# fjdf/slaMEM

Measured on AMD Instinct MI355X. Metric: MEMs/sec (and queries/sec) on 100 Mbp ref x 10 M 150 bp queries, l=20, higher is better.
Workload: dtype u32; 1 GPU; synthetic 100000000 bp reference (splitmix64 seed 42) x 10000000 reads/GPU of 150 bp, 2% substitutions, 50% reverse-complemented, -b -l 20; ref_len=100000000, reads_total=10000000, read_len=150, min_len=20, both_strands=True, parallelism=query shards x1, one GPU, no replication

## Files before the change

### slamem_amd/csrc/mem_search.hip

```cpp
#include "common.h"
#include "prims.h"

#include <atomic>
#include <type_traits>
#include <new>
#include <stdlib.h>
#include <string.h>

namespace slamem {

struct Blk {
    uint4 a;
    uint4 b;
    uint4 c;
    uint4 d;
};

__device__ __forceinline__ uint64_t u64_of(uint32_t lo, uint32_t hi) { return ((uint64_t)hi << 32) | lo; }

__device__ __forceinline__ Blk load_blk(const FMBlock* __restrict__ fm, uint32_t bi) {
    const uint4* p = reinterpret_cast<const uint4*>(fm + bi);
    Blk k;
    k.a = p[0]; k.b = p[1]; k.c = p[2]; k.d = p[3];
    return k;
// ... 1773 lines not shown
    const uint32_t a = sl * kSliceLen;
    if (!(slen >= k && slen - a >= 1u)) return 0;
    const uint32_t b = slen - a < kSliceLen ? slen : a + kSliceLen;
    auto win = [&](uint32_t p, uint32_t len, bool& has_n) -> uint64_t {
        const uint64_t v = span_letters(pk, nm, rel + (rev ? slen - p - len : p), len, has_n);
        if (rev) return ~v & ((1ull << (2u * len)) - 1ull);
        uint64_t r = __brevll(v) >> (64u - 2u * len);
        return ((r & 0x5555555555555555ull) << 1) | ((r >> 1) & 0x5555555555555555ull);
    };
    auto present = [&](const uint64_t* line, uint64_t h) -> bool {
        const uint64_t bits = kfilter_bits(h);
        return (line[kfilter_word(h)] & bits) == bits;
    };
    uint8_t res = 0;
    bool hn;
    if (s <= 6u) {
        const uint32_t k1 = k - 2u, s1 = L - k1 + 1u;
        const bool three = L >= k + 2u && k + 2u <= 32u && ix.kfilter_levels >= 3u;
        const uint32_t p0 = (a + s1 - 1u) / s1 * s1;
        const uint32_t pmax = (uint32_t)(((uint64_t)b + s1 - 2u < (uint64_t)(slen - k1)) ? b + s1 - 2u : slen - k1);
#pragma unroll 1
        for (uint32_t p = p0; p <= pmax && !res; p += s1) {
            const uint64_t v1 = win(p, k1, hn);
            if (hn) { res = 1; break; }
            const uint64_t h1 = kfilter_hash(v1 ^ kFilterShortSalt);
            const uint64_t* line = ix.kfilter + kfilter_line(h1, ix.kfilter_log2);
            if (kStats) n_probe++;
            if (!present(line, h1)) continue;
#pragma unroll 1
            for (uint32_t t = 0; t < 3u && !res; t++) {
                if (p + t < 2u || (uint64_t)p + t - 2u + k > slen) continue;
                const uint32_t q = p + t - 2u;
                const uint64_t vk = win(q, k, hn);
                if (hn) { res = 1; break; }
                if (!present(line, kfilter_hash(vk))) continue;
                if (!three) { res = 1; break; }
#pragma unroll 1
                for (uint32_t u = 0; u < 3u && !res; u++) {
                    if (q + u < 2u || (uint64_t)q + u + k > slen) continue;
                    const uint64_t v3 = win(q + u - 2u, k + 2u, hn);
                    if (hn) { res = 1; break; }
                    if (present(line, kfilter_hash(v3 ^ kFilterLongSalt))) res = 1;
                }
            }
        }
    } else {
        const uint32_t p0 = (a + s - 1u) / s * s;
        const uint32_t pmax = (uint32_t)(((uint64_t)b + s - 2u < (uint64_t)(slen - k)) ? b + s - 2u : slen - k);
#pragma unroll 1
        for (uint32_t p = p0; p <= pmax && !res; p += s) {
            const uint64_t vk = win(p, k, hn);
            if (hn) { res = 1; break; }
            const uint64_t* line = ix.kfilter + kfilter_line(kfilter_hash((vk >> 4) ^ kFilterShortSalt), ix.kfilter_log2);
            if (kStats) n_probe++;
            if (!present(line, kfilter_hash(vk))) continue;
            if (k + 2u > 32u || ix.kfilter_levels < 3u) { res = 1; break; }
#pragma unroll 1
            for (uint32_t u = 0; u < 3u && !res; u++) {
                if (p + u < 2u || (uint64_t)p + u + k > slen) continue;
                const uint64_t v3 = win(p + u - 2u, k + 2u, hn);
                if (hn || present(line, kfilter_hash(v3 ^ kFilterLongSalt))) res = 1;
            }
        }
    }
    return res;
}

template <bool kStats>
__device__ __forceinline__ uint8_t prefilter_item(const SearchArgs& A, const ItemDesc& d, uint32_t& n_probe, uint32_t& n_qload) {
    const IndexView& ix = A.ix;
    const uint32_t k = ix.kfilter_k, L = A.min_len;
    const uint32_t s = L - k + 1u;
    uint32_t sl = d.slice_rev & 0x7FFFFFFFu;
    uint32_t a = sl * kSliceLen;
    uint32_t b = d.len - a < kSliceLen ? d.len : a + kSliceLen;
    uint8_t res = 0;
    if (d.len >= k && d.len - a >= 1u && s <= 6u) {
        const uint32_t k1 = k - 2u, s1 = L - k1 + 1u;
        const uint32_t p0 = (a + s1 - 1u) / s1 * s1;
        uint32_t pmax = (uint32_t)(((uint64_t)b + s1 - 2u < (uint64_t)(d.len - k1)) ? b + s1 - 2u : d.len - k1);
        if (p0 <= pmax) {
            QueryStream qs;
            const bool three = L >= k + 2u && k + 2u <= 32u && ix.kfilter_levels >= 3u;
            const uint32_t kw = three ? k + 2u : k;
            const uint64_t mask = kw >= 32u ? ~0ull : (1ull << (2u * kw)) - 1ull;
            const uint64_t maskk = (1ull << (2u * k)) - 1ull, mask1 = (1ull << (2u * k1)) - 1ull;
            uint64_t km = 0;
            uint32_t run = 0, confirm = 0, confirm2 = 0;
            const uint64_t* line1 = ix.kfilter;
            const uint64_t* line2 = ix.kfilter;
            uint32_t x = p0 >= 4u ? p0 - 4u : 0u;
            qs.init(A.qwords, d.base, d.len, d.slice_rev >> 31, x);
            uint64_t xe64 = (uint64_t)pmax + k1 + 1u + (three ? 2u : 0u);
            const uint32_t xend = xe64 > (uint64_t)d.len - 1u ? d.len - 1u : (uint32_t)xe64;
            uint32_t wend = p0 + k1 - 1u;
            const uint32_t wlast = pmax + k1 - 1u;
            for (; x <= xend && !res; x++) {
                uint32_t c = qs.next();
                if (c >= 2u) { km = ((km << 2) | (uint64_t)(c - 2u)) & mask; run++; }
                else { km = 0; run = 0; }
                if (x == wend && wend <= wlast) {
                    wend += s1;
                    if (run < k1) res = 1;
                    else {
                        uint64_t h = kfilter_hash((km & mask1) ^ kFilterShortSalt), bits = kfilter_bits(h);
                        if (kStats) n_probe++;
                        line1 = ix.kfilter + kfilter_line(h, ix.kfilter_log2);
                        if ((line1[kfilter_word(h)] & bits) == bits) confirm = 3;
                    }
                }
                if (confirm && !res) {
                    confirm--;
                    if (x + 1u >= k) {
                        if (run < k) res = 1;
                        else {
                            uint64_t h = kfilter_hash(km & maskk), bits = kfilter_bits(h);
                            if ((line1[kfilter_word(h)] & bits) == bits) {
                                if (three) { confirm2 = 3; line2 = line1; }
                                else res = 1;
                            }
                        }
                    }
                }
                if (confirm2 && !res) {
                    confirm2--;
                    if (x + 1u >= k + 2u) {
                        if (run < k + 2u) res = 1;
                        else {
                            uint64_t h = kfilter_hash(km ^ kFilterLongSalt), bits = kfilter_bits(h);
                            if ((line2[kfilter_word(h)] & bits) == bits) res = 1;
                        }
                    }
                }
            }
            if (kStats) n_qload += qs.loads;
        }
    } else if (d.len >= k && d.len - a >= 1u) {
        const uint32_t p0 = (a + s - 1u) / s * s;
        const uint32_t pmax = (uint32_t)(((uint64_t)b + s - 2u < (uint64_t)(d.len - k)) ? b + s - 2u : d.len - k);
        if (p0 <= pmax) {
            QueryStream qs;
            qs.init(A.qwords, d.base, d.len, d.slice_rev >> 31, p0);
            const uint64_t mask = (1ull << (2u * k)) - 1ull;
            uint64_t km = 0;
            uint32_t run = 0, wend = p0 + k - 1u;
            const uint32_t xend = pmax + k - 1u;
            for (uint32_t x = p0; x <= xend && !res; x++) {
                uint32_t c = qs.next();
                if (c >= 2u) { km = ((km << 2) | (uint64_t)(c - 2u)) & mask; run++; }
                else { km = 0; run = 0; }
                if (x == wend) {
                    wend += s;
                    if (run < k) res = 1;
                    else {
                        const uint64_t* line = ix.kfilter + kfilter_line(kfilter_hash((km >> 4) ^ kFilterShortSalt), ix.kfilter_log2);
                        uint64_t h = kfilter_hash(km), bits = kfilter_bits(h);
                        if (kStats) n_probe++;
                        if ((line[kfilter_word(h)] & bits) == bits) res = 1;
                    }
                }
            }
            if (kStats) n_qload += qs.loads;
        }
    }
    return res;
}

#ifndef SLAMEM_PF_WAVES
#define SLAMEM_PF_WAVES 8
#endif
template <bool kStats>
__global__ void __launch_bounds__(256, SLAMEM_PF_WAVES) k_prefilter(SearchArgs A, uint8_t* __restrict__ alive) {
    uint64_t g = (uint64_t)blockIdx.x * blockDim.x + threadIdx.x;
    const bool live = g < A.num_items;
    if (!live) g = 0;
    uint32_t n_probe = 0, n_qload = 0;
    ItemDesc d = A.items[g];
    if (!live) d.len = 0;
    uint8_t res;
    if (kPfStageChunks != 0u) {
        __shared__ uint32_t s_pk[kPfStageChunks + 2u];
        __shared__ uint16_t s_nm[kPfStageChunks + 2u];
        __shared__ unsigned long long s_lo[4], s_hi[4];
        unsigned long long lo = d.len ? d.base >> 4 : ~0ull, hi = d.len ? ((d.base + d.len - 1u) >> 4) + 1ull : 0ull;
#pragma unroll
        for (int o = 32; o; o >>= 1) {
            unsigned long long l2 = __shfl_xor(lo, o), h2 = __shfl_xor(hi, o);
            lo = l2 < lo ? l2 : lo;
            hi = h2 > hi ? h2 : hi;
        }
        if ((threadIdx.x & 63u) == 0u) { s_lo[threadIdx.x >> 6] = lo; s_hi[threadIdx.x >> 6] = hi; }
        __syncthreads();
#pragma unroll
        for (int w = 0; w < 4; w++) {
            lo = s_lo[w] < lo ? s_lo[w] : lo;
            hi = s_hi[w] > hi ? s_hi[w] : hi;
        }
        auto pack_span = [&](unsigned long long first_chunk, uint32_t n) {
            const uint4* src = reinterpret_cast<const uint4*>(A.qwords) + first_chunk;
#pragma unroll 1
            for (uint32_t i = threadIdx.x; i < n; i += 256u) {
                uint32_t pk, nm;
                pack_chunk(src[i], pk, nm);
                s_pk[i] = pk;
                s_nm[i] = (uint16_t)nm;
                if (kStats) n_qload++;
            }
            if (threadIdx.x < 2u) { s_pk[n + threadIdx.x] = 0u; s_nm[n + threadIdx.x] = 0u; }
            __syncthreads();
        };
        if (hi > lo && hi - lo <= (unsigned long long)kPfStageChunks) {
            pack_span(lo, (uint32_t)(hi - lo));
            res = prefilter_item_packed<kStats>(A, d, s_pk, s_nm, (uint32_t)(d.base - (lo << 4)), n_probe);
        } else {
            auto span_lo = [&](uint32_t first, uint32_t count) {
                unsigned long long v = ~0ull;
                for (uint32_t w = first; w < first + count; w++) v = s_lo[w] < v ? s_lo[w] : v;
                return v;
            };
            auto span_hi = [&](uint32_t first, uint32_t count) {
                unsigned long long v = 0ull;
                for (uint32_t w = first; w < first + count; w++) v = s_hi[w] > v ? s_hi[w] : v;
                return v;
            };
            uint32_t per_part = 0u;
            for (uint32_t cnt = 2u; cnt >= 1u && !per_part; cnt >>= 1) {
                bool fits = true;
                for (uint32_t first = 0; first < 4u; first += cnt) {
                    const unsigned long long l = span_lo(first, cnt), h = span_hi(first, cnt);
                    if (h > l && h - l > (unsigned long long)kPfStageChunks) fits = false;
                }
                if (fits) per_part = cnt;
            }
            if (per_part && hi > lo) {
                const uint32_t my_wave = threadIdx.x >> 6;
                res = 0;
#pragma unroll 1
                for (uint32_t first = 0; first < 4u; first += per_part) {
                    lo = span_lo(first, per_part);
                    hi = span_hi(first, per_part);
                    if (hi <= lo) continue;
                    __syncthreads();
                    pack_span(lo, (uint32_t)(hi - lo));
                    if (my_wave >= first && my_wave < first + per_part)
                        res = prefilter_item_packed<kStats>(A, d, s_pk, s_nm, (uint32_t)(d.base - (lo << 4)), n_probe);
                }
            } else {
                res = prefilter_item<kStats>(A, d, n_probe, n_qload);
            }
        }
    } else {
        res = prefilter_item<kStats>(A, d, n_probe, n_qload);
    }
    if (live) alive[g] = res;
    if (kStats) {
        stat_flush<kStats>(A.stats + SC_PF_PROBES, n_probe);
        stat_flush<kStats>(A.stats + SC_PF_QUERY_LOADS, n_qload);
        stat_flush<kStats>(A.stats + SC_PF_ITEMS, live ? 1u : 0u);
    }
}

__global__ void __launch_bounds__(256) k_prefilter_list(SearchArgs A, const uint32_t* __restrict__ list, const uint32_t* __restrict__ list_count,
                                                        uint8_t* __restrict__ alive) {
    const uint32_t count = *list_count;
    for (uint32_t i = blockIdx.x * blockDim.x + threadIdx.x; i < count; i += gridDim.x * blockDim.x) {
        const uint32_t g = list[i];
        const ItemDesc d = item_of(A, g);
        uint32_t n_probe = 0, n_qload = 0;
        if (!prefilter_item<false>(A, d, n_probe, n_qload)) alive[g] = 0;
    }
}

#ifndef SLAMEM_SEED_READS
#define SLAMEM_SEED_READS 21
#endif
constexpr uint32_t kSeedReads = SLAMEM_SEED_READS, kSeedReadsMid = 16, kSeedReadsLong = 16;
constexpr uint32_t kSeedMaxLen = 192;
constexpr uint32_t kSeedMaxLenMid = 256;
constexpr uint32_t kSeedMaxLenLong = 384;
#ifndef SLAMEM_SEED_JOBS
#define SLAMEM_SEED_JOBS 16
#endif
constexpr uint32_t kSeedJobs = SLAMEM_SEED_JOBS;
#ifndef SLAMEM_SEED_MEMS
#define SLAMEM_SEED_MEMS 12
#endif
constexpr uint32_t kSeedMems = SLAMEM_SEED_MEMS;
constexpr uint32_t kSigLetters = 12, kSigMask = (1u << kSigLetters) - 1u, kSigKnown = 1u << 24;

template <uint32_t NW, uint32_t R>
struct SeedWave {
    static constexpr uint32_t kJobs = kSeedJobs * R * NW / 3u, kMems = kSeedMems * R * NW / 3u;
    uint64_t pl[R][2][2][NW + 1];
    uint32_t len[R];
    uint32_t nwin[R];
    union {
        uint4 raw[R * NW * 4 + 1];
        struct {
            uint32_t job_p[kJobs], job_x[kJobs];
            uint32_t mem_key[kMems], mem_ref[kMems];
            uint32_t mem_sig[kMems];
        };
    };
    uint32_t bad[R];
    uint64_t pn[R][NW + 1];
    uint32_t hasn;
    unsigned long long expl[R];
    union {
        uint16_t ring[128];
        unsigned long long smask[2 * R];
    };
    uint32_t flags;
    uint32_t pad[3];
};

__device__ __forceinline__ void wave_sync() {
    __builtin_amdgcn_fence(__ATOMIC_RELEASE, "wavefront");
    __builtin_amdgcn_wave_barrier();
    __builtin_amdgcn_fence(__ATOMIC_ACQUIRE, "wavefront");
}
__device__ __forceinline__ uint64_t funnel64(uint64_t lo, uint64_t hi, uint32_t sh) { return (lo >> sh) | ((hi << 1) << (63u - sh)); }
__device__ __forceinline__ uint64_t bits_below(int x) {
    const int c = x < 0 ? 0 : x > 64 ? 64 : x;
    return c == 0 ? 0ull : (~0ull >> (64 - c));
}
__device__ __forceinline__ uint64_t bits_range(int lo, int hi) { return bits_below(hi) & ~bits_below(lo); }
__device__ __forceinline__ uint32_t sel4(const uint4& v, uint32_t a) {
    const uint32_t lo = (a & 1u) ? v.y : v.x, hi = (a & 1u) ? v.w : v.z;
    return (a & 2u) ? hi : lo;
}
__device__ __forceinline__ uint32_t sel12(const uint4& b0, const uint4& b1, const uint4& b2, uint32_t e) {
    const uint32_t a = e & 3u, x0 = sel4(b0, a), x1 = sel4(b1, a), x2 = sel4(b2, a);
    return e < 4u ? x0 : e < 8u ? x1 : x2;
}
__device__ __forceinline__ uint32_t byte_tops(uint32_t m) {
    const uint32_t y = m >> 7;
    return (y | (y >> 7) | (y >> 14) | (y >> 21)) & 0xFu;
}

#ifndef SLAMEM_SEED_WAVES
#define SLAMEM_SEED_WAVES 1
#endif
template <bool kStats, uint32_t NW, uint32_t R>
__global__ void __launch_bounds__(256, SLAMEM_SEED_WAVES) k_seed_mems(SearchArgs A, uint8_t* __restrict__ alive) {
    constexpr uint32_t kMaxLen = 64u * NW;
    static_assert(R <= 32u && R * NW <= 128u, "a flag word holds a bit per read; the planes step runs in at most two passes");
    __shared__ SeedWave<NW, R> lds[4];
    const IndexView& ix = A.ix;
    const uint32_t lane = threadIdx.x & 63u, wv = threadIdx.x >> 6;
    SeedWave<NW, R>& S = lds[wv];
    const uint32_t strands = A.strands, k = ix.seed_k, L = A.min_len, s = L - k + 1u;
    const uint32_t kmask = (1u << k) - 1u;
    const uint64_t r0 = ((uint64_t)blockIdx.x * 4u + wv) * R;
    if (r0 >= (uint64_t)A.num_queries) return;
    const uint32_t nr = (uint64_t)A.num_queries - r0 < R ? (uint32_t)((uint64_t)A.num_queries - r0) : R;
    const unsigned long long below = (1ull << lane) - 1ull;
    const int64_t ulast = (int64_t)text_units(ix.n) - 1;
    uint32_t n_win = 0, n_cmp = 0, n_nm = 0, n_mem = 0;

    const uint64_t off = lane <= nr ? A.offsets[r0 + lane] : 0ull;
    constexpr uint32_t kRawChunks = R * NW * 4u + 1u, kSpecIters = (kRawChunks + 63u) / 64u;
#ifndef SLAMEM_SEED_NO_SPEC
    constexpr bool kSpec = kSpecIters <= 5u;
#else
    constexpr bool kSpec = false;
#endif
    uint4 sv[kSpec ? kSpecIters : 1u];
    uint64_t g0 = 0, len0 = 0;
    bool spec = false;
    if (kSpec) {
        const uint64_t o0 = A.offsets[0], o1 = A.offsets[1], o_end = A.offsets[A.num_queries];
        len0 = o1 - o0;
        g0 = o0 + r0 * len0;
        const uint64_t g1 = g0 + (uint64_t)nr * len0;
        spec = len0 != 0ull && len0 <= (uint64_t)kMaxLen && g1 <= o_end;
        const uint32_t gn = spec ? (uint32_t)(((g1 - 1u) >> 4) - (g0 >> 4) + 1u) : 0u;
        const uint4* src = reinterpret_cast<const uint4*>(A.qwords) + (g0 >> 4);
#pragma unroll
        for (uint32_t j = 0; j < kSpecIters; j++) {
            const uint32_t c = lane + 64u * j;
            sv[j] = c < gn ? src[c] : make_uint4(0, 0, 0, 0);
        }
    }
    const uint64_t offn = __shfl_down(off, 1);
    if (kSpec) spec = spec && __ballot(lane <= nr && off != g0 + (uint64_t)lane * len0) == 0ull;
    uint32_t len = 0, nwin = 0;
    bool left = false;
    if (lane < nr) {
        const uint64_t l64 = offn - off;
        if (l64 > kSliceLen) atomicOr(A.seed_long_flag, 1u);
        if (l64 > kMaxLen) left = l64 >= L; else len = (uint32_t)l64;
        if (len >= L) nwin = (len - k) / s + 1u;
        if (nwin > 64u) { left = true; nwin = 0; }
    }
#ifndef SLAMEM_SEED_NO_FORM_HINT
    const uint32_t lg_grid = 31u - (uint32_t)__clz((int)(gridDim.x | 1u));
    if ((blockIdx.x & ((1u << (lg_grid > 8u ? lg_grid - 8u : 0u)) - 1u)) == 0u) {
        const uint64_t l64 = lane < nr ? offn - off : 0ull;
        if (lane == 0u) atomicAdd(A.seed_wide + 3, nr);
        if (NW < 6u) {
            const bool w4 = NW < 4u && l64 > kMaxLen && l64 <= kSeedMaxLenMid && l64 >= L;
            const bool w6 = l64 > (kMaxLen > kSeedMaxLenMid ? kMaxLen : kSeedMaxLenMid) && l64 <= kSeedMaxLenLong && l64 >= L;
            const uint32_t n4 = (uint32_t)__popcll(__ballot(w4)), n6 = (uint32_t)__popcll(__ballot(w6));
            if (lane == 0u && n4) atomicAdd(A.seed_wide, n4);
            if (lane == 0u && n6) atomicAdd(A.seed_wide + 1, n6);
        }
        if (NW > 3u) {
            const bool needed = l64 > (NW == 4u ? kSeedMaxLen : kSeedMaxLenMid) && l64 <= kMaxLen;
            if (__ballot(needed) != 0ull && lane == 0u) A.seed_wide[2] = 1u;
        }
    }
#endif
    uint32_t wflags = (uint32_t)__ballot(left);
    if (lane == 0u) S.flags = 0u;
    const uint32_t plen = nwin ? len : 0u;
    const uint64_t span0 = u64_of((uint32_t)__builtin_amdgcn_readlane((int)(uint32_t)off, 0), (uint32_t)__builtin_amdgcn_readlane((int)(uint32_t)(off >> 32), 0));
    const uint64_t span1 = u64_of((uint32_t)__builtin_amdgcn_readlane((int)(uint32_t)off, (int)nr), (uint32_t)__builtin_amdgcn_readlane((int)(uint32_t)(off >> 32), (int)nr));
    const uint64_t chunk0 = span0 >> 4;
    const uint32_t nchunks = span1 > span0 ? (uint32_t)(((span1 - 1u) >> 4) - chunk0 + 1u) : 0u;
    const bool staged = nchunks <= kRawChunks;
    if (kSpec && spec) {
#pragma unroll
        for (uint32_t j = 0; j < kSpecIters; j++) {
            const uint32_t c = lane + 64u * j;
            if (c < nchunks) S.raw[c] = sv[kSpec ? j : 0u];
        }
    } else if (staged) {
        const uint4* src = reinterpret_cast<const uint4*>(A.qwords) + chunk0;
        for (uint32_t c = lane; c < nchunks; c += 64u) S.raw[c] = src[c];
    }
    wave_sync();
    if (lane < R) S.bad[lane] = 0u;
    if (lane == 0u) S.hasn = 0u;
    const bool text_pure = ix.num_n == 0u;
    wave_sync();
    const uint32_t* rawwords = reinterpret_cast<const uint32_t*>(S.raw);
    const uint32_t* qw32 = reinterpret_cast<const uint32_t*>(A.qwords);
    const uint64_t qlast32 = ((A.offsets[A.num_queries] + 7ull) >> 3) * 2ull - 1ull;
    constexpr uint32_t kRawLast = (R * NW * 4u + 1u) * 4u - 1u;
    for (uint32_t pb = 0; pb < nr * NW; pb += 64u) {
        const uint32_t pp = pb + lane, i = pp / NW, j = pp % NW;
        const bool on = pp < nr * NW;
        const uint32_t Li = __shfl(plen, (int)(on ? i : 0u));
        const uint64_t base = __shfl(off, (int)(on ? i : 0u));
        if (on && 64u * j < Li) {
            const uint32_t nv = Li - 64u * j < 64u ? Li - 64u * j : 64u;
            const uint64_t a = base + 64u * j;
            const uint32_t sh8 = (uint32_t)(a & 3u);
            uint32_t w[17];
            if (staged) {
                const uint32_t i0 = (uint32_t)((a - (chunk0 << 4)) >> 2);
#pragma unroll
                for (uint32_t t = 0; t < 17u; t++) w[t] = rawwords[i0 + t < kRawLast ? i0 + t : kRawLast];
            } else {
                const uint64_t i0 = a >> 2;
#pragma unroll
                for (uint32_t t = 0; t < 17u; t++) w[t] = qw32[i0 + t < qlast32 ? i0 + t : qlast32];
            }
            uint32_t p0lo = 0, p0hi = 0, p1lo = 0, p1hi = 0, bad = 0;
#pragma unroll
            for (uint32_t t = 0; t < 16u; t++) {
                const uint32_t d = __builtin_amdgcn_alignbyte(w[t + 1u], w[t], sh8);
                const uint32_t nb = nv > 4u * t ? (nv - 4u * t < 4u ? nv - 4u * t : 4u) : 0u;
                const uint32_t M = nb >= 4u ? 0x01010101u : (0x01010101u & ((1u << (8u * nb)) - 1u));
                const uint32_t B0 = d, B1 = d >> 1, B2 = d >> 2, B3 = d >> 3, B4 = d >> 4, B6 = d >> 6, B7 = d >> 7;
                const uint32_t tt = B2 & ~B1, good = (B0 ^ tt) & ~((B4 ^ tt) | B3 | B7) & B6;
                bad |= ~good & M;
                const uint32_t X = ((B1 ^ B2) & M) | ((B2 & M) << 4);
                const uint32_t G = (X | (X >> 7) | (X >> 14) | (X >> 21)) & 0xFFu;
                if (t < 8u) { p0lo |= (G & 0xFu) << (4u * t); p1lo |= (G >> 4) << (4u * t); }
                else { p0hi |= (G & 0xFu) << (4u * (t - 8u)); p1hi |= (G >> 4) << (4u * (t - 8u)); }
            }
            S.pl[i][0][0][j] = u64_of(p0lo, p0hi);
            S.pl[i][0][1][j] = u64_of(p1lo, p1hi);
            uint32_t nlo = 0, nhi = 0;
            if (bad && text_pure) {
#pragma unroll
                for (uint32_t t = 0; t < 16u; t++) {
                    const uint32_t d = __builtin_amdgcn_alignbyte(w[t + 1u], w[t], sh8);
                    const uint32_t nb = nv > 4u * t ? (nv - 4u * t < 4u ? nv - 4u * t : 4u) : 0u;
                    const uint32_t M = nb >= 4u ? 0x01010101u : (0x01010101u & ((1u << (8u * nb)) - 1u));
                    const uint32_t B0 = d, B1 = d >> 1, B2 = d >> 2, B3 = d >> 3, B4 = d >> 4, B6 = d >> 6, B7 = d >> 7;
                    const uint32_t tt = B2 & ~B1, X = ~((B0 ^ tt) & ~((B4 ^ tt) | B3 | B7) & B6) & M;
                    const uint32_t G = (X | (X >> 7) | (X >> 14) | (X >> 21)) & 0xFu;
                    if (t < 8u) nlo |= G << (4u * t); else nhi |= G << (4u * (t - 8u));
                }
                S.hasn = 1u;
            } else if (bad) S.bad[i] = 1u;
            S.pn[i][j] = u64_of(nlo, nhi);
        } else if (on) {
            S.pl[i][0][0][j] = 0ull; S.pl[i][0][1][j] = 0ull; S.pn[i][j] = 0ull;
        }
        if (on && j == 0u) { S.pl[i][0][0][NW] = 0ull; S.pl[i][0][1][NW] = 0ull; S.pl[i][1][0][NW] = 0ull; S.pl[i][1][1][NW] = 0ull; S.pn[i][NW] = 0ull; }
    }
    wave_sync();
    for (uint32_t pb = 0; pb < nr * NW; pb += 64u) {
        const uint32_t pp = pb + lane, i = pp / NW, w = pp % NW;
        const bool on = pp < nr * NW;
        const uint32_t Li = __shfl(plen, (int)(on ? i : 0u));
        if (on) {
            const uint32_t sh = kMaxLen - Li, q = sh >> 6, r = sh & 63u;
#pragma unroll
            for (uint32_t pl = 0; pl < 2u; pl++) {
                const uint64_t* f = S.pl[i][0][pl];
                const uint64_t lo = w + q < NW ? __brevll(f[NW - 1u - (w + q)]) : 0ull, hi = w + q + 1u < NW ? __brevll(f[NW - 2u - (w + q)]) : 0ull;
                S.pl[i][1][pl][w] = Li ? ~funnel64(lo, hi, r) & bits_range(0, (int)Li - 64 * (int)w) : 0ull;
            }
        }
    }
    {
        const bool isbad = lane < nr && plen != 0u && S.bad[lane] != 0u;
        wflags |= (uint32_t)__ballot(isbad);
        if (isbad) nwin = 0;
        if (lane < nr) { S.len[lane] = nwin ? len : 0u; S.nwin[lane] = nwin; }
    }
    if (lane == 0u)
        for (uint32_t i = nr; i < R; i++) { S.len[i] = 0u; S.nwin[i] = 0u; }
    wave_sync();
    const uint32_t mfit = k / s > 6u ? 6u : k / s;
    const uint32_t mstep = A.seed_step ? A.seed_step : mfit >= 3u ? mfit : s <= 12u ? 2u : 1u;

    const bool wave_hasn = __builtin_amdgcn_readfirstlane((int)S.hasn) != 0;
    uint32_t lg_slots = 0;
    {
        const uint32_t nwl = lane < nr ? S.nwin[lane] : 0u;
#pragma unroll
        for (uint32_t t = 1, lg = 1; t <= 32u; t <<= 1, lg++)
            if (__ballot(nwl > t) != 0ull) lg_slots = lg;
    }
    if (lane < R) S.expl[lane] = 0ull;
    uint32_t njobs = 0, nmems = 0;

    auto search = [&](auto with_n) {
    constexpr bool hasn = decltype(with_n)::value;
    auto trip = [&](uint32_t ent, bool act, uint32_t step) {
        const uint32_t rs = ent >> 8, wi = ent & 0xFFu;
        const uint32_t Lr = act ? S.len[rs] : 0u;
        const uint32_t o = wi * s;
        uint32_t want = 0, pal = 0;
        uint4 b0 = make_uint4(0, 0, 0, 0), b1 = b0, b2 = b0, b3 = b0;
        if (hasn && act) {
            const uint64_t* PN = S.pn[rs];
            if (((uint32_t)funnel64(PN[o >> 6], PN[(o >> 6) + 1u], o & 63u) & kmask) != 0u) act = false;
        }
        if (act) {
            const uint32_t q = o >> 6, sh = o & 63u;
            const uint64_t* P0 = S.pl[rs][0][0];
            const uint64_t* P1 = S.pl[rs][0][1];
            const uint32_t f0 = (uint32_t)funnel64(P0[q], P0[q + 1u], sh) & kmask, f1 = (uint32_t)funnel64(P1[q], P1[q + 1u], sh) & kmask;
            uint32_t bucket, tagbits, orient;
            seed_place(f0, f1, k, ix.seed_log2, bucket, tagbits, orient, pal);
            want = tagbits | (orient << 7);
            const uint4* B = reinterpret_cast<const uint4*>(ix.seed + bucket);
            b0 = B[0]; b1 = B[1]; b2 = B[2]; b3 = B[3];
        }
        if (kStats) n_win += (uint32_t)__popcll(__ballot(act));
        const uint32_t wbytes = want * 0x01010101u;
        const uint32_t x0 = b3.x ^ wbytes, x1 = b3.y ^ wbytes, x2 = b3.z ^ wbytes;
        const uint32_t m0 = ~((x0 & 0x7F7F7F7Fu) + 0x7F7F7F7Fu) & 0x80808080u, m1 = ~((x1 & 0x7F7F7F7Fu) + 0x7F7F7F7Fu) & 0x80808080u,
                       m2 = ~((x2 & 0x7F7F7F7Fu) + 0x7F7F7F7Fu) & 0x80808080u;
        const uint32_t count = b3.w;
        uint32_t hits = byte_tops(m0) | (byte_tops(m1) << 4) | (byte_tops(m2) << 8);
        const uint32_t rev = byte_tops(x0 & 0x80808080u) | (byte_tops(x1 & 0x80808080u) << 4) | (byte_tops(x2 & 0x80808080u) << 8);
        hits &= count >= kSeedSlots ? 0xFFFu : (1u << count) - 1u;
        if (strands == 1u && step == 1u) hits &= ~rev;
        if (!act) hits = 0;
        const uint32_t xn = act && (count & kSeedSpilled) ? (count >> 24) & 0x1Fu : 0u, xo = (count & 0xFFFFFFu) << 2;
        if (act && count > kSeedSlots && !(count & kSeedSpilled)) {
            atomicOr(&S.flags, 1u << rs);
            if (kStats) atomicAdd(A.stats + SC_SEED_WHY + 1u, 1ull);
            hits = 0;
        }
        const bool both = pal != 0u && strands == 2u;
        if (kStats && both && hits) atomicAdd(A.stats + SC_SEED_WHY + 2u, 1ull);
        const uint32_t e1 = hits ? (uint32_t)__ffs((int)hits) - 1u : 0u;
        const uint32_t p1 = sel12(b0, b1, b2, e1);
        const uint32_t st1 = (rev >> e1) & 1u;
        const uint32_t dist = step * s;
        uint32_t pn = 0, pp1 = 0, ps1 = 0;
        if (dist <= k) {
            pp1 = __shfl_up(p1, 1);
            ps1 = __shfl_up(hits ? st1 : 2u, 1);
            const uint32_t pent = __shfl_up(act ? ent : 0xFFFFFFFFu, 1);
            pn = (lane == 0u || wi < step || pent != ent - step || ps1 == 2u) ? 0u : 1u;
        }
        const uint32_t njobs0 = njobs;
        auto push = [&](bool hv, uint32_t p, uint32_t st) {
            const uint32_t w = st ? p + dist : p - dist;
            const bool job = hv && !(pn && pp1 == w && ps1 == st);
            const unsigned long long qb = __ballot(job);
            const uint32_t at = njobs + (uint32_t)__popcll(qb & below);
            if (job && at < SeedWave<NW, R>::kJobs) {
                S.job_p[at] = p;
                S.job_x[at] = (st ? Lr - k - o : o) | (st << 15) | (rs << 16);
            }
            njobs += (uint32_t)__popcll(qb);
        };
        uint32_t rem = hits;
        for (uint32_t it = 0; __ballot(rem != 0u) != 0ull; it++) {
            const bool hv = rem != 0u;
            const uint32_t e = it == 0u ? e1 : hv ? (uint32_t)__ffs((int)rem) - 1u : 0u;
            rem &= rem - 1u;
            const uint32_t p = it == 0u ? p1 : sel12(b0, b1, b2, e);
            push(hv, p, (rev >> e) & 1u);
            if (__ballot(hv && both) != 0ull) push(hv && both, p, 1u);
        }
        for (uint32_t e0 = 0; __ballot(e0 < xn) != 0ull; e0 += 4u) {
            const bool on = e0 < xn;
            uint4 v0 = make_uint4(0, 0, 0, 0), v1 = v0;
            if (on) {
                const uint4* P = reinterpret_cast<const uint4*>(ix.spill + xo + e0);
                v0 = P[0]; v1 = P[1];
            }
#pragma unroll
            for (uint32_t q = 0; q < 4u; q++) {
                const uint32_t p = q == 0u ? v0.x : q == 1u ? v0.z : q == 2u ? v1.x : v1.z;
                const uint32_t d = ((q == 0u ? v0.y : q == 1u ? v0.w : q == 2u ? v1.y : v1.w) ^ want) & 0xFFu;
                const uint32_t st = d >> 7;
                const bool hv = on && e0 + q < xn && (d & 0x7Fu) == 0u && !(strands == 1u && st && step == 1u);
                if (__ballot(hv) == 0ull) continue;
                push(hv, p, st);
                if (__ballot(hv && both) != 0ull) push(hv && both, p, 1u);
            }
        }
        if (njobs > SeedWave<NW, R>::kJobs) {
            if (act) atomicOr(&S.flags, 1u << rs);
            if (kStats && lane == 0u) atomicAdd(A.stats + SC_SEED_WHY + 3u, 1ull);
            njobs = njobs0;
        }
    };
    auto lookups = [&](uint32_t round) {
        const uint32_t step = round == 0u ? mstep : 1u;
        uint32_t cnt = 0;
        const uint32_t per = 64u >> lg_slots, wi = lane & ((1u << lg_slots) - 1u);
        const uint32_t wmod = wi - mstep * ((wi * (65536u / mstep + 1u)) >> 16);
        for (uint32_t r = 0;; r += per) {
            if (r < nr) {
                const uint32_t rr = r + (lane >> lg_slots);
                const uint32_t nw = (rr >= nr || ((S.flags >> rr) & 1u)) ? 0u : S.nwin[rr];
                const bool pred = wi < nw && (round == 0u ? wmod == 0u : wmod != 0u && ((S.expl[rr] >> wi) & 1ull) == 0ull);
                const unsigned long long pm = __ballot(pred);
                if (pred) S.ring[cnt + (uint32_t)__popcll(pm & below)] = (uint16_t)((rr << 8) | wi);
                cnt += (uint32_t)__popcll(pm);
            }
            const bool last = r >= nr;
            if (cnt >= 64u || (last && cnt != 0u)) {
                wave_sync();
                const bool act = lane < cnt;
                const uint32_t ent = act ? S.ring[lane] : 0u;
                const uint32_t over = lane + 64u < cnt ? S.ring[lane + 64u] : 0u;
                wave_sync();
                if (lane + 64u < cnt) S.ring[lane] = (uint16_t)over;
                cnt = cnt > 64u ? cnt - 64u : 0u;
                trip(ent, act, step);
            }
            if (last) break;
        }
        wave_sync();
    };

    auto compares = [&](uint32_t round) {
        const bool mark = round == 0u && mstep > 1u;
        const uint32_t ms = mstep * s;
        const uint32_t gone = S.flags;
        for (uint32_t jb = 0; jb < njobs; jb += 64u) {
            const bool listed = jb + lane < njobs;
            const uint32_t p = listed ? S.job_p[jb + lane] : 0u, xx = listed ? S.job_x[jb + lane] : 0u;
            const uint32_t os = xx & 0x7FFFu, st = (xx >> 15) & 1u, jr = xx >> 16;
            const bool has = listed && ((gone >> jr) & 1u) == 0u;
            const uint32_t Lj = S.len[jr];
            const int64_t d = (int64_t)p - (int64_t)os;
            const int64_t u0 = d >> 6;
            const uint32_t sh = (uint32_t)(d & 63);
            bool is_mem = false;
            uint32_t key = 0, ref = 0, sig = 0;
            if (has) {
                constexpr int NU = (int)NW + 1;
                int64_t ui[NU];
#pragma unroll
                for (int i = 0; i < NU; i++) { const int64_t u = u0 + i; ui[i] = u < 0 ? 0 : u > ulast ? ulast : u; }
                const uint4* T = reinterpret_cast<const uint4*>(ix.tpl);
                uint4 tu[NU], tx[NU];
#pragma unroll
                for (int i = 0; i < NU; i++) { tu[i] = T[2 * ui[i]]; tx[i] = T[2 * ui[i] + 1]; }
                uint64_t uq[NU], nu[NU];
                uint32_t anyn = 0;
#pragma unroll
                for (int i = 0; i < NU; i++) { nu[i] = u64_of(tx[i].x, tx[i].y); uq[i] = u64_of(tx[i].z, tx[i].w); anyn |= (tx[i].x | tx[i].y); }
                if (kStats && anyn) n_nm++;
                const uint64_t* R0 = S.pl[jr][st][0];
                const uint64_t* R1 = S.pl[jr][st][1];
                uint64_t mm[NW];
#pragma unroll
                for (int w = 0; w < (int)NW; w++)
                    mm[w] = (funnel64(u64_of(tu[w].x, tu[w].y), u64_of(tu[w + 1].x, tu[w + 1].y), sh) ^ R0[w]) |
                            (funnel64(u64_of(tu[w].z, tu[w].w), u64_of(tu[w + 1].z, tu[w + 1].w), sh) ^ R1[w]) | funnel64(nu[w], nu[w + 1], sh);
                if (hasn) {
                    const uint64_t* PN = S.pn[jr];
                    if (st == 0u) {
#pragma unroll
                        for (int w = 0; w < (int)NW; w++) mm[w] |= PN[w];
                    } else {
                        const uint32_t shn = kMaxLen - Lj, qn = shn >> 6, rn = shn & 63u;
#pragma unroll
                        for (int w = 0; w < (int)NW; w++) {
                            const uint32_t x = (uint32_t)w + qn;
                            const uint64_t lo64 = x < NW ? __brevll(PN[NW - 1u - x]) : 0ull, hi64 = x + 1u < NW ? __brevll(PN[NW - 2u - x]) : 0ull;
                            mm[w] |= funnel64(lo64, hi64, rn);
                        }
                    }
                }
                const int lo = d < 0 ? (int)(-d) : 0;
                const int64_t room = (int64_t)ix.n - d;
                const int hi = room < (int64_t)Lj ? (int)room : (int)Lj;
#pragma unroll
                for (int w = 0; w < (int)NW; w++) mm[w] |= ~bits_range(lo - 64 * w, hi - 64 * w);
                uint32_t a = 0, b = kMaxLen;
                bool broken = false;
#pragma unroll
                for (int w = 0; w < (int)NW; w++) {
                    const uint64_t lw = mm[w] & bits_range(0, (int)os - 64 * w);
                    if (lw) a = 64u * w + 64u - (uint32_t)__clzll((long long)lw);
                    if (mm[w] & bits_range((int)os - 64 * w, (int)(os + k) - 64 * w)) broken = true;
                }
#pragma unroll
                for (int w = (int)NW - 1; w >= 0; w--) {
                    const uint64_t hw = mm[w] & ~bits_range(0, (int)(os + k) - 64 * w);
                    if (hw) b = 64u * w + (uint32_t)__ffsll((unsigned long long)hw) - 1u;
                }
                const uint32_t af = st ? Lj - b : a, bf = st ? Lj - a : b, of = st ? Lj - k - os : os;
                bool owner;
                if (round == 0u) owner = !(of >= ms && of - ms >= af);
                else {
                    const uint32_t oa = (af + ms - 1u) / ms * ms;
                    owner = !(mstep > 1u && oa + k <= bf) && !(of >= s && of - s >= af);
                }
                if (broken) {
                    atomicOr(&S.flags, 1u << jr);
                    if (kStats) atomicAdd(A.stats + SC_SEED_WHY + 4u, 1ull);
                }
                else if (owner && b - a >= L && (strands == 2u || st == 0u)) {
                    is_mem = true; key = (a << 16) | (b - a); ref = (uint32_t)(d + (int64_t)a);
                    if (!anyn && b + kSigLetters <= kMaxLen && d + (int64_t)b + (int64_t)kSigLetters <= (int64_t)ix.n) {
                        const uint32_t wb = b >> 6, sb = b & 63u;
                        uint64_t l0 = 0, h0 = 0, l1 = 0, h1 = 0;
#pragma unroll
                        for (int w = 0; w < (int)NW; w++) {
                            const uint64_t t0 = funnel64(u64_of(tu[w].x, tu[w].y), u64_of(tu[w + 1].x, tu[w + 1].y), sh);
                            const uint64_t t1 = funnel64(u64_of(tu[w].z, tu[w].w), u64_of(tu[w + 1].z, tu[w + 1].w), sh);
                            if ((uint32_t)w == wb) { l0 = t0; l1 = t1; }
                            if ((uint32_t)w == wb + 1u) { h0 = t0; h1 = t1; }
                        }
                        sig = kSigKnown | ((uint32_t)funnel64(l0, h0, sb) & kSigMask) | (((uint32_t)funnel64(l1, h1, sb) & kSigMask) << kSigLetters);
                    }
                }
                if (mark && !broken && bf >= af + k) {
                    uint64_t uqs[NW];
#pragma unroll
                    for (int w = 0; w < (int)NW; w++) uqs[w] = funnel64(uq[w], uq[w + 1], sh);
                    unsigned long long done = 0ull;
                    for (uint32_t wi = (af + s - 1u) / s, wl = (bf - k) / s; wi <= wl; wi++) {
                        const uint32_t x = st ? Lj - k - wi * s : wi * s;
                        uint64_t word = 0ull;
#pragma unroll
                        for (int w = 0; w < (int)NW; w++) word = (x >> 6) == (uint32_t)w ? uqs[w] : word;
                        if ((word >> (x & 63u)) & 1ull) done |= 1ull << wi;
                    }
                    if (done) atomicOr(&S.expl[jr], done);
                }
            }
            if (kStats) {
                const uint32_t nh = (uint32_t)__popcll(__ballot(has));
                n_cmp += nh;
                if (mark && lane == 0u) atomicAdd(A.stats + SC_SEED_ONCE, (unsigned long long)nh);
            }
            const unsigned long long mb = __ballot(is_mem);
            if (is_mem) {
                const uint32_t at = nmems + (uint32_t)__popcll(mb & below);
                if (at < SeedWave<NW, R>::kMems) { S.mem_key[at] = key; S.mem_ref[at] = ref; S.mem_sig[at] = sig | ((2u * jr + st) << 25); }
                else { atomicOr(&S.flags, 1u << jr); if (kStats) atomicAdd(A.stats + SC_SEED_WHY + 5u, 1ull); }
            }
            nmems += (uint32_t)__popcll(mb);
        }
        wave_sync();
    };

    for (uint32_t round = 0; round < (mstep > 1u ? 2u : 1u); round++) {
        njobs = 0;
        lookups(round);
        compares(round);
    }
    };
    if (wave_hasn) search(std::true_type{}); else search(std::false_type{});
    {
        if (nmems > SeedWave<NW, R>::kMems) nmems = SeedWave<NW, R>::kMems;

        const uint32_t g0 = (uint32_t)(r0 * strands);
        auto rank_of = [&](uint32_t mi, uint32_t key, uint32_t g, uint32_t& rank, uint32_t& cnt, bool& tie) {
            rank = 0; cnt = 0; tie = false;
            for (uint32_t t2 = 0; t2 < nmems; t2++) {
                const uint32_t kk = S.mem_key[t2], gg = S.mem_sig[t2] >> 25;
                const bool same = gg == g;
                cnt += same ? 1u : 0u;
                rank += (same && kk > key) ? 1u : 0u;
                tie = tie || (same && kk == key && t2 != mi);
            }
        };
        auto tie_rank = [&](uint32_t mi, uint32_t key, uint32_t myref, uint32_t g, uint32_t sig, uint32_t& rank) -> bool {
            const uint32_t a = key >> 16, b = a + (key & 0xFFFFu);
            bool child = false;
            for (uint32_t t2 = 0; t2 < nmems; t2++) {
                const uint32_t kk = S.mem_key[t2], a2 = kk >> 16, b2 = a2 + (kk & 0xFFFFu);
                child = child || ((S.mem_sig[t2] >> 25) == g && kk != key && a2 <= a && b2 > b);
            }
            const uint32_t jr = g >> 1, st = g & 1u;
            uint32_t qb = 0;
            if (child) qb = (uint32_t)((S.pl[jr][st][0][b >> 6] >> (b & 63u)) & 1ull) | ((uint32_t)((S.pl[jr][st][1][b >> 6] >> (b & 63u)) & 1ull) << 1);
            auto letter = [&](uint32_t sg, uint32_t t) { return ((sg >> t) & 1u) | (((sg >> (t + kSigLetters)) & 1u) << 1); };
            const bool rows = ix.prec != nullptr;
            const uint32_t my_side = child && letter(sig, 0u) > qb ? 1u : 0u;
            bool bad = (sig & kSigKnown) == 0u && (child || !rows);
            for (uint32_t t2 = 0; t2 < nmems; t2++) {
                const uint32_t so = S.mem_sig[t2];
                if (t2 == mi || (so >> 25) != g || S.mem_key[t2] != key) continue;
                const bool known = (so & sig & kSigKnown) != 0u;
                if (!known && (child || !rows)) { bad = true; continue; }
                const uint32_t o_side = child && letter(so, 0u) > qb ? 1u : 0u;
                bool before;
                if (o_side != my_side) before = o_side == 0u;
                else {
                    const uint32_t x = sig ^ so, diff = known ? (x | (x >> kSigLetters)) & kSigMask : 0u;
                    bool smaller;
                    if (diff != 0u) {
                        const uint32_t t = (uint32_t)__ffs((int)diff) - 1u;
                        smaller = letter(so, t) < letter(sig, t);
                    } else if (rows) smaller = ix.prec[S.mem_ref[t2]].row < ix.prec[myref].row;
                    else { bad = true; continue; }
                    before = my_side == 0u ? smaller : !smaller;
                }
                rank += before ? 1u : 0u;
            }
            return bad;
        };
        auto emit_mem = [&](uint32_t fl, uint32_t key, uint32_t ref, uint32_t gb, uint32_t rank, uint32_t cnt) {
            if ((fl >> (gb >> 1)) & 1u) return;
            const uint32_t g = g0 + (strands == 2u ? gb : gb >> 1);
            emit3_at(A, g, rank, 0u, ref, key >> 16, (key & 0xFFFFu) | 0x80000000u);
            if (rank == 0u) A.block_counts[g] = cnt;
            if (kStats) n_mem++;
        };
        if (nmems <= 64u) {
            const bool has = lane < nmems;
            const uint32_t key = has ? S.mem_key[lane] : 0u, ref = has ? S.mem_ref[lane] : 0u, g = has ? S.mem_sig[lane] >> 25 : 0xFFFFFFFFu;
            if (lane < 2u * R) S.smask[lane] = 0ull;
            wave_sync();
            if (has) atomicOr(&S.smask[g], 1ull << lane);
            wave_sync();
            const unsigned long long mine = has ? S.smask[g] : 0ull;
            uint32_t rank = 0;
            const uint32_t cnt = (uint32_t)__popcll(mine);
            bool tie = false;
            for (unsigned long long o = mine & ~(1ull << lane); __ballot(o != 0ull) != 0ull; o &= o - 1ull) {
                if (o == 0ull) continue;
                const uint32_t kk = S.mem_key[__ffsll(o) - 1];
                rank += kk > key ? 1u : 0u;
                tie = tie || kk == key;
            }
            if (has && tie && tie_rank(lane, key, ref, g, S.mem_sig[lane], rank)) {
                atomicOr(&S.flags, 1u << (g >> 1));
                if (kStats) atomicAdd(A.stats + SC_SEED_WHY + 6u, 1ull);
            }
            wave_sync();
            if (has) emit_mem(S.flags | wflags, key, ref, g, rank, cnt);
        } else {
            for (uint32_t pass = 0; pass < 2u; pass++) {
                const uint32_t fl = pass ? (S.flags | wflags) : 0u;
                for (uint32_t m0i = 0; m0i < nmems; m0i += 64u) {
                    const uint32_t mi = m0i + lane;
                    const bool has = mi < nmems;
                    const uint32_t key = has ? S.mem_key[mi] : 0u, ref = has ? S.mem_ref[mi] : 0u, g = has ? S.mem_sig[mi] >> 25 : 0xFFFFFFFFu;
                    uint32_t rank, cnt;
                    bool tie;
                    rank_of(mi, key, g, rank, cnt, tie);
                    const bool bad = has && tie && tie_rank(mi, key, ref, g, S.mem_sig[mi], rank);
                    if (!pass) { if (bad) atomicOr(&S.flags, 1u << (g >> 1)); }
                    else if (has) emit_mem(fl, key, ref, g, rank, cnt);
                }
                wave_sync();
            }
        }
    }
    wave_sync();
    const uint32_t fl = S.flags | wflags;
    {
        const bool isleft = lane < nr * strands && ((fl >> (strands == 2u ? lane >> 1 : lane)) & 1u) != 0u;
        if (lane < nr * strands) alive[r0 * strands + lane] = isleft ? 1 : 0;
        const unsigned long long lm = __ballot(isleft);
        if (lm != 0ull) {
            unsigned int at = 0;
            if (lane == 0u) at = atomicAdd(A.seed_left_count, (unsigned int)__popcll(lm));
            at = (unsigned int)__builtin_amdgcn_readfirstlane((int)at);
            if (isleft) A.seed_left_ids[at + (uint32_t)__popcll(lm & below)] = (uint32_t)(r0 * strands + lane);
        }
    }
    if (kStats) {
        stat_flush<kStats>(A.stats + SC_SEED_NMASKS, n_nm);
        stat_flush<kStats>(A.stats + SC_SEED_MEMS, n_mem);
        if (lane == 0u) {
            atomicAdd(A.stats + SC_SEED_WINDOWS, (unsigned long long)n_win);
            atomicAdd(A.stats + SC_SEED_COMPARES, (unsigned long long)n_cmp);
            atomicAdd(A.stats + SC_SEED_READS, (unsigned long long)nr);
            atomicAdd(A.stats + SC_SEED_QBYTES, (unsigned long long)(__builtin_amdgcn_readlane((int)(uint32_t)off, (int)nr) - __builtin_amdgcn_readlane((int)(uint32_t)off, 0)));
            atomicAdd(A.stats + SC_SEED_LEFT, (unsigned long long)(strands * (uint32_t)__popc(fl)));
            atomicAdd(A.stats + SC_SEED_WHY + 0u, (unsigned long long)__popc(wflags));
        }
    }
}

__global__ void __launch_bounds__(256) k_place_inline(const RawRow* __restrict__ inl, uint64_t stride, const uint32_t* __restrict__ counts,
                                                      const uint64_t* __restrict__ item_off, uint64_t nitems,
                                                      const uint32_t* __restrict__ sa, uint64_t capacity,
                                                      slamem_mem* __restrict__ out, const uint8_t* __restrict__ inline_valid) {
    uint64_t g = (uint64_t)blockIdx.x * blockDim.x + threadIdx.x;
    if (g >= nitems) return;
    uint32_t cnt = counts[g];
    uint64_t off = item_off[g];
    uint32_t iv = inline_valid ? inline_valid[g] : 0u;
    asm volatile("" : "+v"(cnt), "+v"(off), "+v"(iv));
    if (cnt > kInlineMems) cnt = kInlineMems;
    if (iv && cnt > iv - 1u) cnt = iv - 1u;
    if (cnt == 0u) return;
    static_assert(kInlineMems == 4, "k_place_inline is written for four inline slots");
    const RawRow* in = inl + g;
    const RawRow none = {0u, 0u, 0x80000000u};
    RawRow r0 = in[0], r1 = none, r2 = none, r3 = none;
    if (cnt > 1u) r1 = in[stride];
    if (cnt > 2u) r2 = in[2u * stride];
    if (cnt > 3u) r3 = in[3u * stride];
    asm volatile("" : "+v"(r0.row), "+v"(r0.pos), "+v"(r0.len), "+v"(r1.row), "+v"(r1.pos), "+v"(r1.len));
    asm volatile("" : "+v"(r2.row), "+v"(r2.pos), "+v"(r2.len), "+v"(r3.row), "+v"(r3.pos), "+v"(r3.len));
    uint32_t p0 = r0.row, p1 = r1.row, p2 = r2.row, p3 = r3.row;
    if (!(r0.len >> 31)) p0 = sa[r0.row];
    if (cnt > 1u && !(r1.len >> 31)) p1 = sa[r1.row];
    if (cnt > 2u && !(r2.len >> 31)) p2 = sa[r2.row];
    if (cnt > 3u && !(r3.len >> 31)) p3 = sa[r3.row];
    asm volatile("" : "+v"(p0), "+v"(p1), "+v"(p2), "+v"(p3));
    if (off < capacity) out[off] = slamem_mem{p0, r0.pos, r0.len & 0x7FFFFFFFu};
    if (cnt > 1u && off + 1u < capacity) out[off + 1u] = slamem_mem{p1, r1.pos, r1.len & 0x7FFFFFFFu};
    if (cnt > 2u && off + 2u < capacity) out[off + 2u] = slamem_mem{p2, r2.pos, r2.len & 0x7FFFFFFFu};
    if (cnt > 3u && off + 3u < capacity) out[off + 3u] = slamem_mem{p3, r3.pos, r3.len & 0x7FFFFFFFu};
}

__global__ void __launch_bounds__(256) k_group_totals(const uint32_t* __restrict__ counts, uint64_t nitems, uint64_t* __restrict__ totals) {
    const uint64_t g = (uint64_t)blockIdx.x * blockDim.x + threadIdx.x;
    uint64_t v = g < nitems ? (uint64_t)counts[g] : 0ull;
#pragma unroll
    for (int d = 32; d > 0; d >>= 1) v += u64_of(__shfl_down((uint32_t)v, d), __shfl_down((uint32_t)(v >> 32), d));
    if ((threadIdx.x & 63u) == 0u && (g >> 6) <= (nitems >> 6)) totals[g >> 6] = v;
}
__global__ void __launch_bounds__(256) k_place_grouped(const uint32_t* __restrict__ counts, uint64_t nitems, const uint64_t* __restrict__ group_prefix,
                                                       uint64_t* __restrict__ block_offsets, const RawRow* __restrict__ inl, uint64_t stride,
                                                       const uint32_t* __restrict__ sa, uint64_t capacity, slamem_mem* __restrict__ out,
                                                       const uint8_t* __restrict__ inline_valid) {
    const uint64_t g = (uint64_t)blockIdx.x * blockDim.x + threadIdx.x;
    const uint32_t lane = threadIdx.x & 63u;
    const bool item = g < nitems;
    const uint32_t full = item ? counts[g] : 0u;
    uint32_t iv = (item && inline_valid) ? inline_valid[g] : 0u;
    uint64_t gp = g <= nitems ? group_prefix[g >> 6] : 0ull;
    RawRow r0 = {0u, 0u, 0x80000000u};
    if (full != 0u) r0 = inl[g];
    asm volatile("" : "+v"(iv), "+v"(gp), "+v"(r0.row), "+v"(r0.pos), "+v"(r0.len));
    uint64_t incl = full;
#pragma unroll
    for (int d = 1; d < 64; d <<= 1) {
        const uint64_t o = u64_of(__shfl_up((uint32_t)incl, d), __shfl_up((uint32_t)(incl >> 32), d));
        if ((int)lane >= d) incl += o;
    }
    const uint64_t off = gp + (incl - full);
    if (g <= nitems) block_offsets[g] = off;
    uint32_t cnt = full > kInlineMems ? kInlineMems : full;
    if (iv && cnt > iv - 1u) cnt = iv - 1u;
    if (cnt == 0u) return;
    static_assert(kInlineMems == 4, "k_place_grouped is written for four inline slots");
    const RawRow none = {0u, 0u, 0x80000000u};
    RawRow r1 = none, r2 = none, r3 = none;
    if (cnt > 1u) r1 = inl[stride + g];
    if (cnt > 2u) r2 = inl[2u * stride + g];
    if (cnt > 3u) r3 = inl[3u * stride + g];
    asm volatile("" : "+v"(r1.row), "+v"(r1.pos), "+v"(r1.len), "+v"(r2.row), "+v"(r2.pos), "+v"(r2.len), "+v"(r3.row), "+v"(r3.pos), "+v"(r3.len));
    uint32_t p0 = r0.row, p1 = r1.row, p2 = r2.row, p3 = r3.row;
    if (!(r0.len >> 31)) p0 = sa[r0.row];
    if (cnt > 1u && !(r1.len >> 31)) p1 = sa[r1.row];
    if (cnt > 2u && !(r2.len >> 31)) p2 = sa[r2.row];
    if (cnt > 3u && !(r3.len >> 31)) p3 = sa[r3.row];
    asm volatile("" : "+v"(p0), "+v"(p1), "+v"(p2), "+v"(p3));
    if (off < capacity) out[off] = slamem_mem{p0, r0.pos, r0.len & 0x7FFFFFFFu};
    if (cnt > 1u && off + 1u < capacity) out[off + 1u] = slamem_mem{p1, r1.pos, r1.len & 0x7FFFFFFFu};
    if (cnt > 2u && off + 2u < capacity) out[off + 2u] = slamem_mem{p2, r2.pos, r2.len & 0x7FFFFFFFu};
    if (cnt > 3u && off + 3u < capacity) out[off + 3u] = slamem_mem{p3, r3.pos, r3.len & 0x7FFFFFFFu};
}

__global__ void __launch_bounds__(256) k_place_overflow(const RawKey* __restrict__ key, const slamem_mem* __restrict__ raw,
                                                        const unsigned long long* __restrict__ listed,
                                                        const uint64_t* __restrict__ item_off,
                                                        const uint8_t* __restrict__ item_attempt,
                                                        const uint32_t* __restrict__ sa, uint64_t capacity,
                                                        slamem_mem* __restrict__ out, const uint32_t* __restrict__ raw_seg,
                                                        const uint32_t* __restrict__ pool) {
    uint64_t count = *listed;
    if (count > capacity) count = capacity;
    const uint64_t stride = (uint64_t)gridDim.x * blockDim.x;
    for (uint64_t i = (uint64_t)blockIdx.x * blockDim.x + threadIdx.x; i < count; i += stride) {
        RawKey kk = key[i];
        if (kk.block == 0xFFFFFFFFu) continue;
        if ((kk.k >> 28) != item_attempt[kk.block]) continue;
        slamem_mem m = raw[i];
        uint64_t pos = item_off[kk.block] + (kk.k & 0x0FFFFFFFu);
        if (raw_seg) {
            const uint32_t sg = raw_seg[i];
            if (sg != 0xFFFFFFFFu) pos += pool[sg];
        }
        if (pos >= capacity) continue;
        if (m.length >> 31) m.length &= 0x7FFFFFFFu;
        else m.ref_pos = sa[m.ref_pos];
        out[pos] = m;
    }
}

__global__ void __launch_bounds__(256) k_item_counts(const uint64_t* __restrict__ offsets, uint32_t nq, uint32_t slice_len,
                                                     uint32_t* __restrict__ cnt, uint32_t* __restrict__ wps,
                                                     unsigned int* __restrict__ most) {
    uint64_t q = (uint64_t)blockIdx.x * blockDim.x + threadIdx.x;
    uint32_t c = 0, w = 0;
    if (q < nq) {
        uint64_t len = offsets[q + 1] - offsets[q];
        c = slice_len ? (uint32_t)((len + slice_len - 1) / slice_len) : 1u;
        if (c == 0) c = 1;
        w = 2u * (uint32_t)((len + 31u) >> 5);
    }
    if (c > 1u) atomicMax(most, c);
    if (q > nq) return;
    cnt[q] = c;
    wps[q] = w;
}

__global__ void __launch_bounds__(256) k_item_fill(const uint64_t* __restrict__ offsets, const uint32_t* __restrict__ first,
                                                   const uint64_t* __restrict__ wscan, uint32_t nq, uint32_t strands,
                                                   ItemDesc* __restrict__ items, uint64_t* __restrict__ item_pk,
                                                   uint32_t* __restrict__ item_block) {
    uint64_t q = (uint64_t)blockIdx.x * blockDim.x + threadIdx.x;
    if (q >= nq) return;
    uint64_t o0 = offsets[q];
    uint32_t len = (uint32_t)(offsets[q + 1] - o0);
    uint32_t f = first[q], cnt = first[q + 1] - f;
    uint64_t w0 = wscan ? wscan[q] : 0ull, wps = wscan ? wscan[q + 1] - w0 : 0ull;
    for (uint32_t s = 0; s < strands; s++)
        for (uint32_t c = 0; c < cnt; c++) {
            uint64_t it = (uint64_t)strands * f + (uint64_t)s * cnt + (cnt - 1u - c);
            items[it] = ItemDesc{o0, len, c | (s << 31)};
            if (item_pk) item_pk[it] = 2ull + (uint64_t)strands * w0 + (uint64_t)s * wps;
            if (item_block) item_block[it] = (uint32_t)(q * strands + s);
        }
}

__global__ void __launch_bounds__(256) k_block_offsets(const uint32_t* __restrict__ first, const uint64_t* __restrict__ item_off,
                                                       uint32_t nq, uint32_t strands, uint64_t nitems,
                                                       uint64_t* __restrict__ block_offsets) {
    uint64_t b = (uint64_t)blockIdx.x * blockDim.x + threadIdx.x;
    uint64_t nblocks = (uint64_t)nq * strands;
    if (b > nblocks) return;
// ... 956 lines not shown
```

Measured before the change: 4.518 billion MEMs/s.

## Mark explained seeds with per-position bitmaps and clip match bounds arithmetically

Replaces the per-read window-index bitmask with a per-position bitmap per read (mark[R][NW]). Unique-position words are OR'd in word-wise, reversing the bits for the reverse strand, instead of looping over each window and selecting a word. Also packs the per-read bad flags into one atomic bitmask and clamps a/b to the valid reference range after the mismatch scan, rather than OR-ing range masks into every mismatch word. It aims to cut per-lane loop and select work in the seed marking pass, at the cost of more LDS for the mark array and extra atomics.

New measurement: 4.638 billion MEMs/s (median of 6 runs). +2.6%, better.

```diff
diff --git a/slamem_amd/csrc/mem_search.hip b/slamem_amd/csrc/mem_search.hip
--- a/slamem_amd/csrc/mem_search.hip
+++ b/slamem_amd/csrc/mem_search.hip
@@ -2099,16 +2099,15 @@
             uint32_t mem_sig[kMems];
         };
     };
-    uint32_t bad[R];
+    uint32_t bad;
     uint64_t pn[R][NW + 1];
     uint32_t hasn;
-    unsigned long long expl[R];
+    unsigned long long mark[R][NW];
     union {
         uint16_t ring[128];
         unsigned long long smask[2 * R];
     };
     uint32_t flags;
-    uint32_t pad[3];
 };
 
 __device__ __forceinline__ void wave_sync() {
@@ -2227,8 +2226,7 @@
         for (uint32_t c = lane; c < nchunks; c += 64u) S.raw[c] = src[c];
     }
     wave_sync();
-    if (lane < R) S.bad[lane] = 0u;
-    if (lane == 0u) S.hasn = 0u;
+    if (lane == 0u) { S.bad = 0u; S.hasn = 0u; }
     const bool text_pure = ix.num_n == 0u;
     wave_sync();
     const uint32_t* rawwords = reinterpret_cast<const uint32_t*>(S.raw);
@@ -2283,7 +2281,7 @@
                     if (t < 8u) nlo |= G << (4u * t); else nhi |= G << (4u * (t - 8u));
                 }
                 S.hasn = 1u;
-            } else if (bad) S.bad[i] = 1u;
+            } else if (bad) atomicOr(&S.bad, 1u << i);
             S.pn[i][j] = u64_of(nlo, nhi);
         } else if (on) {
             S.pl[i][0][0][j] = 0ull; S.pl[i][0][1][j] = 0ull; S.pn[i][j] = 0ull;
@@ -2306,7 +2304,7 @@
         }
     }
     {
-        const bool isbad = lane < nr && plen != 0u && S.bad[lane] != 0u;
+        const bool isbad = lane < nr && plen != 0u && ((S.bad >> lane) & 1u) != 0u;
         wflags |= (uint32_t)__ballot(isbad);
         if (isbad) nwin = 0;
         if (lane < nr) { S.len[lane] = nwin ? len : 0u; S.nwin[lane] = nwin; }
@@ -2325,7 +2323,7 @@
         for (uint32_t t = 1, lg = 1; t <= 32u; t <<= 1, lg++)
             if (__ballot(nwl > t) != 0ull) lg_slots = lg;
     }
-    if (lane < R) S.expl[lane] = 0ull;
+    for (uint32_t c = lane; c < R * NW; c += 64u) (&S.mark[0][0])[c] = 0ull;
     uint32_t njobs = 0, nmems = 0;
 
     auto search = [&](auto with_n) {
@@ -2435,7 +2433,9 @@
             if (r < nr) {
                 const uint32_t rr = r + (lane >> lg_slots);
                 const uint32_t nw = (rr >= nr || ((S.flags >> rr) & 1u)) ? 0u : S.nwin[rr];
-                const bool pred = wi < nw && (round == 0u ? wmod == 0u : wmod != 0u && ((S.expl[rr] >> wi) & 1ull) == 0ull);
+                const bool mine = wi < nw && (round == 0u ? wmod == 0u : wmod != 0u);
+                const uint32_t wo = mine ? wi * s : 0u;
+                const bool pred = mine && (round == 0u || ((reinterpret_cast<const uint32_t*>(S.mark[mine ? rr : 0u])[wo >> 5] >> (wo & 31u)) & 1u) == 0u);
                 const unsigned long long pm = __ballot(pred);
                 if (pred) S.ring[cnt + (uint32_t)__popcll(pm & below)] = (uint16_t)((rr << 8) | wi);
                 cnt += (uint32_t)__popcll(pm);
@@ -2485,6 +2485,10 @@
 #pragma unroll
                 for (int i = 0; i < NU; i++) { nu[i] = u64_of(tx[i].x, tx[i].y); uq[i] = u64_of(tx[i].z, tx[i].w); anyn |= (tx[i].x | tx[i].y); }
                 if (kStats && anyn) n_nm++;
+                if (mark) {
+#pragma unroll
+                    for (int w = 0; w < (int)NW; w++) uq[w] = funnel64(uq[w], uq[w + 1], sh);
+                }
                 const uint64_t* R0 = S.pl[jr][st][0];
                 const uint64_t* R1 = S.pl[jr][st][1];
                 uint64_t mm[NW];
@@ -2510,8 +2514,6 @@
                 const int lo = d < 0 ? (int)(-d) : 0;
                 const int64_t room = (int64_t)ix.n - d;
                 const int hi = room < (int64_t)Lj ? (int)room : (int)Lj;
-#pragma unroll
-                for (int w = 0; w < (int)NW; w++) mm[w] |= ~bits_range(lo - 64 * w, hi - 64 * w);
                 uint32_t a = 0, b = kMaxLen;
                 bool broken = false;
 #pragma unroll
@@ -2525,6 +2527,9 @@
                     const uint64_t hw = mm[w] & ~bits_range(0, (int)(os + k) - 64 * w);
                     if (hw) b = 64u * w + (uint32_t)__ffsll((unsigned long long)hw) - 1u;
                 }
+                if ((int)a < lo) a = (uint32_t)lo;
+                if ((int)b > hi) b = (uint32_t)hi;
+                broken = broken || (int)os < lo || (int)(os + k) > hi;
                 const uint32_t af = st ? Lj - b : a, bf = st ? Lj - a : b, of = st ? Lj - k - os : os;
                 bool owner;
                 if (round == 0u) owner = !(of >= ms && of - ms >= af);
@@ -2552,18 +2557,24 @@
                     }
                 }
                 if (mark && !broken && bf >= af + k) {
-                    uint64_t uqs[NW];
+                    auto once = [&](int w) { return uq[w] & bits_range((int)a - 64 * w, (int)(b - k) + 1 - 64 * w); };
+                    if (st) {
+                        const uint32_t shm = kMaxLen - 1u - Lj + k, qm = shm >> 6, rm = shm & 63u;
+                        uint64_t cur = __brevll(once((int)NW - 1));
 #pragma unroll
-                    for (int w = 0; w < (int)NW; w++) uqs[w] = funnel64(uq[w], uq[w + 1], sh);
-                    unsigned long long done = 0ull;
-                    for (uint32_t wi = (af + s - 1u) / s, wl = (bf - k) / s; wi <= wl; wi++) {
-                        const uint32_t x = st ? Lj - k - wi * s : wi * s;
-                        uint64_t word = 0ull;
+                        for (int v = 0; v < (int)NW; v++) {
+                            const uint64_t next = v + 1 < (int)NW ? __brevll(once((int)NW - 2 - v)) : 0ull;
+                            const uint64_t f = funnel64(cur, next, rm);
+                            if (f != 0ull && (uint32_t)v >= qm) atomicOr(&S.mark[jr][(uint32_t)v - qm], f);
+                            cur = next;
+                        }
+                    } else {
 #pragma unroll
-                        for (int w = 0; w < (int)NW; w++) word = (x >> 6) == (uint32_t)w ? uqs[w] : word;
-                        if ((word >> (x & 63u)) & 1ull) done |= 1ull << wi;
+                        for (int w = 0; w < (int)NW; w++) {
+                            const uint64_t f = once(w);
+                            if (f != 0ull) atomicOr(&S.mark[jr][w], f);
+                        }
                     }
-                    if (done) atomicOr(&S.expl[jr], done);
                 }
             }
             if (kStats) {
```
